# cgranerob/Land-Surface-Temperature-Super-Resolution-with-a-Scale-Invariance-Free-Neural-Approach

Measured on AMD Instinct MI355X. Metric: LST+NDVI 256x256 patches/sec (train fwd+bwd), whole job, higher is better.
Workload: dtype f32; 1 GPU; ModelB SIF-NN-SR2 (gradFTM loss) batch 64/GPU, synthetic 256x256, 1x MI355X, fwd+loss+bwd+Adam; batch_per_gpu=64, patch=256x256 (LST 64x64 + NDVI 256x256), parallelism=dp1, loss=sr2

## Files before the change

land-surface-temperature-super-resolution-with-a-scale-invariance-free-neural-approach_amd/csrc/resample.hip:

```cpp
#include "edge_conv.h"

namespace {

__device__ __forceinline__ float4 maybe_bnrelu(float4 v, const float* scale, const float* shift, int c) {
  return scale != nullptr ? bn_relu4(v, ld4(scale + c), ld4(shift + c)) : v;
}

template <bool HS>
__global__ void bnrelu_pool2_kernel(const float* __restrict__ y, const float* scale, const float* shift,
                                    float* __restrict__ out, int B, int H, int W, int C) {
  const unsigned Q = C / 4, Ho = H / 2, Wo = W / 2;
  const unsigned n = (unsigned)B * Ho * Wo * Q;
  for (unsigned e = blockIdx.x * blockDim.x + threadIdx.x; e < n; e += gridDim.x * blockDim.x) {
    const unsigned p = e / Q;
    const int c = (int)(e - p * Q) * 4;
    const unsigned rr = p / Wo, ox = p - rr * Wo, b = rr / Ho, oy = rr - b * Ho;
    const size_t s = (((size_t)b * H + 2 * oy) * W + 2 * ox) * C + c;
    const float4 v00 = maybe_bnrelu(ldA4<HS>(y, s), scale, shift, c), v01 = maybe_bnrelu(ldA4<HS>(y, s + C), scale, shift, c);
    const float4 v10 = maybe_bnrelu(ldA4<HS>(y, s + (size_t)W * C), scale, shift, c);
    const float4 v11 = maybe_bnrelu(ldA4<HS>(y, s + (size_t)W * C + C), scale, shift, c);
    float4 o;
    o.x = (v00.x + v01.x + v10.x + v11.x) * 0.25f;
    o.y = (v00.y + v01.y + v10.y + v11.y) * 0.25f;
    o.z = (v00.z + v01.z + v10.z + v11.z) * 0.25f;
    o.w = (v00.w + v01.w + v10.w + v11.w) * 0.25f;
    stA4<HS>(out, (size_t)p * C + c, o);
  }
}

template <bool HS>
__global__ void bnrelu_add_kernel(const float* __restrict__ p, const float* __restrict__ y, const float* scale,
                                  const float* shift, float* __restrict__ out, int C, size_t nquads) {
  const unsigned Q = C / 4;
  for (size_t e = (size_t)blockIdx.x * blockDim.x + threadIdx.x; e < nquads; e += (size_t)gridDim.x * blockDim.x) {
    const int c = (int)((unsigned)e % Q) * 4;
    const float4 a = ldA4<HS>(p, e * 4), v = maybe_bnrelu(ldA4<HS>(y, e * 4), scale, shift, c);
    stA4<HS>(out, e * 4, make_float4(a.x + v.x, a.y + v.y, a.z + v.z, a.w + v.w));
  }
}

__device__ __forceinline__ void up_coord(int o, int in, int out, int& i0, int& i1, float& l0, float& l1) {
#pragma clang fp contract(off)
  const float ratio = out > 1 ? (float)(in - 1) / (float)(out - 1) : 0.f;
  const float src = ratio * (float)o;
  i0 = (int)src;
  i1 = i0 + (i0 < in - 1 ? 1 : 0);
  l1 = src - (float)i0;
  l0 = 1.f - l1;
}

template <bool HS>
__global__ void bnrelu_up2x_kernel(const float* __restrict__ y, const float* scale, const float* shift,
                                   float* __restrict__ out, int B, int Hin, int Win, int C) {
  const int Q = C / 4, Ho = 2 * Hin, Wo = 2 * Win;
  const size_t n = (size_t)B * Ho * Wo * Q;
  for (size_t e = (size_t)blockIdx.x * blockDim.x + threadIdx.x; e < n; e += (size_t)gridDim.x * blockDim.x) {
    const int c = (int)(e % Q) * 4;
    const size_t p = e / Q;
    const int ox = p % Wo, oy = (p / Wo) % Ho, b = p / ((size_t)Wo * Ho);
    int y0, y1, x0, x1; float hy0, hy1, hx0, hx1;
    up_coord(oy, Hin, Ho, y0, y1, hy0, hy1);
    up_coord(ox, Win, Wo, x0, x1, hx0, hx1);
    const size_t base = (size_t)b * Hin * Win * C + c;
    const float4 v00 = maybe_bnrelu(ldA4<HS>(y, base + ((size_t)y0 * Win + x0) * C), scale, shift, c);
    const float4 v01 = maybe_bnrelu(ldA4<HS>(y, base + ((size_t)y0 * Win + x1) * C), scale, shift, c);
    const float4 v10 = maybe_bnrelu(ldA4<HS>(y, base + ((size_t)y1 * Win + x0) * C), scale, shift, c);
    const float4 v11 = maybe_bnrelu(ldA4<HS>(y, base + ((size_t)y1 * Win + x1) * C), scale, shift, c);
    float4 o;
    o.x = hy0 * (hx0 * v00.x + hx1 * v01.x) + hy1 * (hx0 * v10.x + hx1 * v11.x);
    o.y = hy0 * (hx0 * v00.y + hx1 * v01.y) + hy1 * (hx0 * v10.y + hx1 * v11.y);
    o.z = hy0 * (hx0 * v00.z + hx1 * v01.z) + hy1 * (hx0 * v10.z + hx1 * v11.z);
    o.w = hy0 * (hx0 * v00.w + hx1 * v01.w) + hy1 * (hx0 * v10.w + hx1 * v11.w);
    stA4<HS>(out, p * C + c, o);
  }
}

template <bool HS>
__global__ void pool2_bwd_kernel(const float* __restrict__ gp, float* __restrict__ g, int B, int H, int W, int C,
                                 int accumulate) {
  const int Q = C / 4, Ho = H / 2, Wo = W / 2;
  const size_t n = (size_t)B * H * W * Q;
  for (size_t e = (size_t)blockIdx.x * blockDim.x + threadIdx.x; e < n; e += (size_t)gridDim.x * blockDim.x) {
    const int c = (int)(e % Q) * 4;
    const size_t p = e / Q;
    const int x = p % W, yy = (p / W) % H, b = p / ((size_t)W * H);
    const float4 v = ldA4<HS>(gp, (((size_t)b * Ho + yy / 2) * Wo + x / 2) * C + c);
    float4 o = make_float4(0.25f * v.x, 0.25f * v.y, 0.25f * v.z, 0.25f * v.w);
    if (accumulate) {
      const float4 a = ldA4<HS>(g, p * C + c);
      o.x += a.x; o.y += a.y; o.z += a.z; o.w += a.w;
    }
    stA4<HS>(g, p * C + c, o);
  }
}

template <bool HS>
__global__ void up2x_bwd_kernel(const float* __restrict__ gu, float* __restrict__ g, int B, int Hin, int Win, int C) {
  SIFSR_CHAIN_PRIO();
  const int Q = C / 4, Ho = 2 * Hin, Wo = 2 * Win;
  const size_t n = (size_t)B * Hin * Win * Q;
  for (size_t e = (size_t)blockIdx.x * blockDim.x + threadIdx.x; e < n; e += (size_t)gridDim.x * blockDim.x) {
    const int c = (int)(e % Q) * 4;
    const size_t p = e / Q;
    const int ix = p % Win, iy = (p / Win) % Hin, b = p / ((size_t)Win * Hin);
    float wy[5], wx[5];
#pragma unroll
    for (int k = 0; k < 5; ++k) {
      const int oy = 2 * iy - 2 + k, ox = 2 * ix - 2 + k;
      wy[k] = 0.f; wx[k] = 0.f;
      if (oy >= 0 && oy < Ho) {
        int a0, a1; float l0, l1;
        up_coord(oy, Hin, Ho, a0, a1, l0, l1);
        wy[k] = (a0 == iy ? l0 : 0.f) + (a1 == iy ? l1 : 0.f);
      }
      if (ox >= 0 && ox < Wo) {
        int a0, a1; float l0, l1;
        up_coord(ox, Win, Wo, a0, a1, l0, l1);
        wx[k] = (a0 == ix ? l0 : 0.f) + (a1 == ix ? l1 : 0.f);
      }
    }
    float4 acc = make_float4(0.f, 0.f, 0.f, 0.f);
#pragma unroll
    for (int ky = 0; ky < 5; ++ky) {
      if (wy[ky] == 0.f) continue;
      const int oy = 2 * iy - 2 + ky;
#pragma unroll
      for (int kx = 0; kx < 5; ++kx) {
        if (wx[kx] == 0.f) continue;
        const int ox = 2 * ix - 2 + kx;
        const float w = wy[ky] * wx[kx];
        const float4 v = ldA4<HS>(gu, (((size_t)b * Ho + oy) * Wo + ox) * C + c);
        acc.x = fmaf(w, v.x, acc.x); acc.y = fmaf(w, v.y, acc.y); acc.z = fmaf(w, v.z, acc.z); acc.w = fmaf(w, v.w, acc.w);
      }
    }
    stA4<HS>(g, p * C + c, acc);
  }
}

template <int C, bool HS>
__global__ __launch_bounds__(256) void bnrelu_up2x_tile_kernel(const float* __restrict__ y, const float* scale,
                                                               const float* shift, float* __restrict__ out, int Hin,
                                                               int Win) {
  constexpr int Q = C / 4, SR = 10;
  __shared__ float4 src[SR * SR * Q];
  const int tid = threadIdx.x;
  const int Ho = 2 * Hin, Wo = 2 * Win;
  const int ox0 = blockIdx.x * 16, oy0 = blockIdx.y * 16, b = blockIdx.z;
  int sy0, sx0, t1; float f0, f1;
  up_coord(oy0, Hin, Ho, sy0, t1, f0, f1);
  up_coord(ox0, Win, Wo, sx0, t1, f0, f1);
  for (int e = tid; e < SR * SR * Q; e += 256) {
    const int c4 = e % Q, p = e / Q;
    const int py = p / SR, px = p - py * SR;
    const int gy = min(sy0 + py, Hin - 1), gx = min(sx0 + px, Win - 1);
    src[e] = maybe_bnrelu(ldA4<HS>(y, ((size_t)(b * Hin + gy) * Win + gx) * C + 4 * c4), scale, shift, 4 * c4);
  }
  __syncthreads();
  for (int e = tid; e < 256 * Q; e += 256) {
    const int c4 = e % Q, p = e / Q;
    const int oy = oy0 + (p >> 4), ox = ox0 + (p & 15);
    if (oy >= Ho || ox >= Wo) continue;
    int y0, y1, x0, x1; float hy0, hy1, hx0, hx1;
    up_coord(oy, Hin, Ho, y0, y1, hy0, hy1);
    up_coord(ox, Win, Wo, x0, x1, hx0, hx1);
    const float4 v00 = src[((y0 - sy0) * SR + (x0 - sx0)) * Q + c4], v01 = src[((y0 - sy0) * SR + (x1 - sx0)) * Q + c4];
    const float4 v10 = src[((y1 - sy0) * SR + (x0 - sx0)) * Q + c4], v11 = src[((y1 - sy0) * SR + (x1 - sx0)) * Q + c4];
    float4 o;
    o.x = hy0 * (hx0 * v00.x + hx1 * v01.x) + hy1 * (hx0 * v10.x + hx1 * v11.x);
    o.y = hy0 * (hx0 * v00.y + hx1 * v01.y) + hy1 * (hx0 * v10.y + hx1 * v11.y);
    o.z = hy0 * (hx0 * v00.z + hx1 * v01.z) + hy1 * (hx0 * v10.z + hx1 * v11.z);
    o.w = hy0 * (hx0 * v00.w + hx1 * v01.w) + hy1 * (hx0 * v10.w + hx1 * v11.w);
    stA4<HS>(out, ((size_t)(b * Ho + oy) * Wo + ox) * C + 4 * c4, o);
  }
}

template <int C, bool HS>
__global__ __launch_bounds__(256) void up2x_bwd_tile_kernel(const float* __restrict__ gu, float* __restrict__ g, int Hin,
                                                            int Win, const float* __restrict__ bn_y,
                                                            const float* __restrict__ bn_scale,
                                                            const float* __restrict__ bn_shift,
                                                            float* __restrict__ bn_partials) {
  SIFSR_CHAIN_PRIO();
  constexpr int TL = 8, HR = 2 * TL + 3, NCH = C / 16;
  __shared__ float4 hi[HR * HR * 4];
  __shared__ float4 tmp[HR * TL * 4];
  __shared__ float wxs[TL][5], wys[TL][5];
  const int tid = threadIdx.x;
  const int Ho = 2 * Hin, Wo = 2 * Win;
  const int ix0 = blockIdx.x * TL, iy0 = blockIdx.y * TL;
  const int b = blockIdx.z / NCH, ch0 = (blockIdx.z % NCH) * 16;
  if (tid < 2 * TL * 5) {
    const bool isy = tid >= TL * 5;
    const int t = isy ? tid - TL * 5 : tid;
    const int il = t / 5, k = t - il * 5;
    const int i = (isy ? iy0 : ix0) + il, in = isy ? Hin : Win, on = isy ? Ho : Wo;
    const int o = 2 * i - 2 + k;
    float w = 0.f;
    if (i < in && o >= 0 && o < on) {
      int a0, a1; float l0, l1;
      up_coord(o, in, on, a0, a1, l0, l1);
      w = (a0 == i ? l0 : 0.f) + (a1 == i ? l1 : 0.f);
    }
    if (isy) wys[il][k] = w; else wxs[il][k] = w;
  }
  for (int e = tid; e < HR * HR * 4; e += 256) {
    const int q = e & 3, p = e >> 2;
    const int py = p / HR, px = p - py * HR;
    const int oy = 2 * iy0 - 2 + py, ox = 2 * ix0 - 2 + px;
    float4 v = make_float4(0.f, 0.f, 0.f, 0.f);
    if (oy >= 0 && oy < Ho && ox >= 0 && ox < Wo) v = ldA4<HS>(gu, ((size_t)(b * Ho + oy) * Wo + ox) * C + ch0 + 4 * q);
    hi[e] = v;
  }
  __syncthreads();
  for (int e = tid; e < HR * TL * 4; e += 256) {
    const int q = e & 3, p = e >> 2;
    const int py = p / TL, il = p - py * TL;
    float4 acc = make_float4(0.f, 0.f, 0.f, 0.f);
#pragma unroll
    for (int k = 0; k < 5; ++k) {
      const float w = wxs[il][k];
      const float4 v = hi[(py * HR + 2 * il + k) * 4 + q];
      acc.x = fmaf(w, v.x, acc.x); acc.y = fmaf(w, v.y, acc.y); acc.z = fmaf(w, v.z, acc.z); acc.w = fmaf(w, v.w, acc.w);
    }
    tmp[e] = acc;
  }
  __syncthreads();
  {
    const int q = tid & 3, p = tid >> 2;
    const int il_y = p / TL, il_x = p - il_y * TL;
    const int iy = iy0 + il_y, ix = ix0 + il_x;
    float4 acc = make_float4(0.f, 0.f, 0.f, 0.f);
#pragma unroll
    for (int k = 0; k < 5; ++k) {
      const float w = wys[il_y][k];
      const float4 v = tmp[((2 * il_y + k) * TL + il_x) * 4 + q];
      acc.x = fmaf(w, v.x, acc.x); acc.y = fmaf(w, v.y, acc.y); acc.z = fmaf(w, v.z, acc.z); acc.w = fmaf(w, v.w, acc.w);
    }
    const bool in = iy < Hin && ix < Win;
    acc = as_stored4<HS>(acc);
    if (in) stA4<HS>(g, ((size_t)(b * Hin + iy) * Win + ix) * C + ch0 + 4 * q, acc);
    if (bn_partials != nullptr) {
      float4 d1 = make_float4(0.f, 0.f, 0.f, 0.f), d2 = d1;
      if (in) {
        const float4 yv = ldA4<HS>(bn_y, ((size_t)(b * Hin + iy) * Win + ix) * C + ch0 + 4 * q);
        const float4 sc = ld4(bn_scale + ch0 + 4 * q), sh = ld4(bn_shift + ch0 + 4 * q);
        d1.x = fmaf(yv.x, sc.x, sh.x) > 0.f ? acc.x : 0.f; d2.x = d1.x * yv.x;
        d1.y = fmaf(yv.y, sc.y, sh.y) > 0.f ? acc.y : 0.f; d2.y = d1.y * yv.y;
        d1.z = fmaf(yv.z, sc.z, sh.z) > 0.f ? acc.z : 0.f; d2.z = d1.z * yv.z;
        d1.w = fmaf(yv.w, sc.w, sh.w) > 0.f ? acc.w : 0.f; d2.w = d1.w * yv.w;
      }
      float v8[8] = {d1.x, d1.y, d1.z, d1.w, d2.x, d2.y, d2.z, d2.w};
#pragma unroll
      for (int m = 4; m < 64; m <<= 1)
#pragma unroll
        for (int j = 0; j < 8; ++j) v8[j] += __shfl_xor(v8[j], m);
      __syncthreads();
      float* const red = reinterpret_cast<float*>(hi);
      if ((tid & 63) < 4) {
#pragma unroll
        for (int j = 0; j < 8; ++j) red[((tid >> 6) * 4 + (tid & 3)) * 8 + j] = v8[j];
      }
      __syncthreads();
      if (tid < 32) {
        const int qq = tid & 3, r = (tid >> 2) & 3, which = tid >> 4;
        const float sum = (red[(0 * 4 + qq) * 8 + which * 4 + r] + red[(1 * 4 + qq) * 8 + which * 4 + r]) +
                          (red[(2 * 4 + qq) * 8 + which * 4 + r] + red[(3 * 4 + qq) * 8 + which * 4 + r]);
        const size_t row = ((size_t)b * gridDim.y + blockIdx.y) * gridDim.x + blockIdx.x;
        bn_partials[(row * C + ch0 + 4 * qq + r) * 2 + which] = sum;
      }
    }
  }
}

inline int grid_for(size_t n) {
  size_t b = (n + 255) / 256;
  return (int)(b > 16384 ? 16384 : (b < 1 ? 1 : b));
}

}

int launch_bnrelu_pool2(const float* y, const float* scale, const float* shift, float* out, int B, int H, int W, int C, hipStream_t s) {
  if (H % 2 || W % 2 || C % 4 || (size_t)B * H * W * C >= ((size_t)1 << 32)) return SIFSR_ERR_SHAPE;
  if (sifsr_half_storage()) hipLaunchKernelGGL(bnrelu_pool2_kernel<true>, dim3(grid_for((size_t)B * H / 2 * W / 2 * C / 4)), dim3(256), 0, s, y, scale, shift, out, B, H, W, C);
  else hipLaunchKernelGGL(bnrelu_pool2_kernel<false>, dim3(grid_for((size_t)B * H / 2 * W / 2 * C / 4)), dim3(256), 0, s, y, scale, shift, out, B, H, W, C);
  SIFSR_LAUNCH_CHECK();
  return SIFSR_OK;
}
int launch_bnrelu_add(const float* p, const float* y, const float* scale, const float* shift, float* out, int C, size_t npix, hipStream_t s) {
  if (C % 4) return SIFSR_ERR_SHAPE;
  const size_t nq = npix * C / 4;
  if (sifsr_half_storage()) hipLaunchKernelGGL(bnrelu_add_kernel<true>, dim3(grid_for(nq)), dim3(256), 0, s, p, y, scale, shift, out, C, nq);
  else hipLaunchKernelGGL(bnrelu_add_kernel<false>, dim3(grid_for(nq)), dim3(256), 0, s, p, y, scale, shift, out, C, nq);
  SIFSR_LAUNCH_CHECK();
  return SIFSR_OK;
}
int launch_bnrelu_up2x(const float* y, const float* scale, const float* shift, float* out, int B, int Hin, int Win, int C, hipStream_t s) {
  if (C % 4) return SIFSR_ERR_SHAPE;
  if ((C == 16 || C == 32 || C == 64) && B <= 65535 && Hin >= 2 && Win >= 2) {
    const dim3 grid((2 * Win + 15) / 16, (2 * Hin + 15) / 16, B);
#define SIFSR_UP(CV, HV) hipLaunchKernelGGL((bnrelu_up2x_tile_kernel<CV, HV>), grid, dim3(256), 0, s, y, scale, shift, out, Hin, Win)
    const bool hs = sifsr_half_storage();
    if (C == 16) { if (hs) SIFSR_UP(16, true); else SIFSR_UP(16, false); }
    else if (C == 32) { if (hs) SIFSR_UP(32, true); else SIFSR_UP(32, false); }
    else { if (hs) SIFSR_UP(64, true); else SIFSR_UP(64, false); }
#undef SIFSR_UP
    SIFSR_LAUNCH_CHECK();
    return SIFSR_OK;
  }
  if (sifsr_half_storage()) hipLaunchKernelGGL(bnrelu_up2x_kernel<true>, dim3(grid_for((size_t)B * Hin * Win * C)), dim3(256), 0, s, y, scale, shift, out, B, Hin, Win, C);
  else hipLaunchKernelGGL(bnrelu_up2x_kernel<false>, dim3(grid_for((size_t)B * Hin * Win * C)), dim3(256), 0, s, y, scale, shift, out, B, Hin, Win, C);
  SIFSR_LAUNCH_CHECK();
  return SIFSR_OK;
}
int launch_pool2_bwd(const float* gp, float* g, int B, int H, int W, int C, int accumulate, hipStream_t s) {
  if (H % 2 || W % 2 || C % 4) return SIFSR_ERR_SHAPE;
  if (sifsr_half_storage()) hipLaunchKernelGGL(pool2_bwd_kernel<true>, dim3(grid_for((size_t)B * H * W * C / 4)), dim3(256), 0, s, gp, g, B, H, W, C, accumulate);
  else hipLaunchKernelGGL(pool2_bwd_kernel<false>, dim3(grid_for((size_t)B * H * W * C / 4)), dim3(256), 0, s, gp, g, B, H, W, C, accumulate);
  SIFSR_LAUNCH_CHECK();
  return SIFSR_OK;
}
int up2x_bwd_stat_rows(int B, int Hin, int Win, int C) {
  if (!((C == 16 || C == 32 || C == 64) && (size_t)B * (C / 16) <= 65535)) return 0;
  return B * ((Hin + 7) / 8) * ((Win + 7) / 8);
}

int launch_up2x_bwd(const float* gu, float* g, int B, int Hin, int Win, int C, hipStream_t s, const float* bn_y,
                    const float* bn_scale, const float* bn_shift, float* bn_partials) {
  if (C % 4) return SIFSR_ERR_SHAPE;
  if (bn_partials != nullptr && (!bn_y || !bn_scale || !bn_shift || up2x_bwd_stat_rows(B, Hin, Win, C) == 0)) return SIFSR_ERR_ARG;
  if ((C == 16 || C == 32 || C == 64) && (size_t)B * (C / 16) <= 65535) {
    const dim3 grid((Win + 7) / 8, (Hin + 7) / 8, B * (C / 16));
#define SIFSR_UPB(CV, HV) hipLaunchKernelGGL((up2x_bwd_tile_kernel<CV, HV>), grid, dim3(256), 0, s, gu, g, Hin, Win, bn_y, bn_scale, bn_shift, bn_partials)
    const bool hs = sifsr_half_storage();
    if (C == 16) { if (hs) SIFSR_UPB(16, true); else SIFSR_UPB(16, false); }
    else if (C == 32) { if (hs) SIFSR_UPB(32, true); else SIFSR_UPB(32, false); }
    else { if (hs) SIFSR_UPB(64, true); else SIFSR_UPB(64, false); }
#undef SIFSR_UPB
    SIFSR_LAUNCH_CHECK();
    return SIFSR_OK;
  }
  if (sifsr_half_storage()) hipLaunchKernelGGL(up2x_bwd_kernel<true>, dim3(grid_for((size_t)B * Hin * Win * C / 4)), dim3(256), 0, s, gu, g, B, Hin, Win, C);
  else hipLaunchKernelGGL(up2x_bwd_kernel<false>, dim3(grid_for((size_t)B * Hin * Win * C / 4)), dim3(256), 0, s, gu, g, B, Hin, Win, C);
  SIFSR_LAUNCH_CHECK();
  return SIFSR_OK;
}
```

Baseline: 10750 patches/s.

## Make up2x backward tile kernel persistent with software-pipelined tile prefetch

```diff
diff --git a/land-surface-temperature-super-resolution-with-a-scale-invariance-free-neural-approach_amd/csrc/resample.hip b/land-surface-temperature-super-resolution-with-a-scale-invariance-free-neural-approach_amd/csrc/resample.hip
--- a/land-surface-temperature-super-resolution-with-a-scale-invariance-free-neural-approach_amd/csrc/resample.hip
+++ b/land-surface-temperature-super-resolution-with-a-scale-invariance-free-neural-approach_amd/csrc/resample.hip
@@ -1,4 +1,6 @@
 #include "edge_conv.h"
+#include <algorithm>
+#include <type_traits>
 
 namespace {
 
@@ -174,102 +176,223 @@
   }
 }
 
-template <int C, bool HS>
-__global__ __launch_bounds__(256) void up2x_bwd_tile_kernel(const float* __restrict__ gu, float* __restrict__ g, int Hin,
-                                                            int Win, const float* __restrict__ bn_y,
-                                                            const float* __restrict__ bn_scale,
-                                                            const float* __restrict__ bn_shift,
-                                                            float* __restrict__ bn_partials) {
-  SIFSR_CHAIN_PRIO();
-  constexpr int TL = 8, HR = 2 * TL + 3, NCH = C / 16;
-  __shared__ float4 hi[HR * HR * 4];
-  __shared__ float4 tmp[HR * TL * 4];
-  __shared__ float wxs[TL][5], wys[TL][5];
+#ifndef SIFSR_UP2X_WGS
+#define SIFSR_UP2X_WGS 1024
+#endif
+#ifndef SIFSR_UP2X_WALK_MIN
+#define SIFSR_UP2X_WALK_MIN 4
+#endif
+#ifndef SIFSR_UP2X_WALK_MAX
+#define SIFSR_UP2X_WALK_MAX 16
+#endif
+#ifndef SIFSR_UP2X_LDS_PAD
+#define SIFSR_UP2X_LDS_PAD 0
+#endif
+
+template <bool HS> struct RawQuad { using type = float4; };
+template <> struct RawQuad<true> { using type = uint2; };
+template <bool HS> static __device__ __forceinline__ typename RawQuad<HS>::type ld_raw4(const float* base, size_t e) {
+  if constexpr (HS) return *reinterpret_cast<const uint2*>(reinterpret_cast<const unsigned short*>(base) + e);
+  else return *reinterpret_cast<const float4*>(base + e);
+}
+template <bool HS> static __device__ __forceinline__ float4 widen4(typename RawQuad<HS>::type r) {
+  if constexpr (HS) return unpack_bf16x4(r); else return r;
+}
+
+static __device__ __forceinline__ int fresh(int v) { asm volatile("" : "+v"(v)); return v; }
+
+template <int C> struct Up2xBwdLds {
+  static constexpr int HI = 6 * 256, TMP = 19 * 8 * 4, YB = 256, BNC = 2 * (C / 4);
+  static constexpr size_t BYTES = (size_t)(HI + TMP + YB + BNC) * sizeof(float4) + (4 * 8 * 5 + 4 * 4 * 8) * sizeof(float);
+};
+
+template <int C, bool HS, bool STATS>
+__device__ __forceinline__ void up2x_bwd_walk(const float* __restrict__ gu, float* __restrict__ g, int Hin, int Win,
+                                              const float* __restrict__ bn_y, const float* __restrict__ bn_scale,
+                                              const float* __restrict__ bn_shift, float* __restrict__ bn_partials,
+                                              int n_items, int walk) {
+  constexpr int TL = 8, HR = 2 * TL + 3, NCH = C / 16, NW = HR * HR * 4, NLD = (NW + 255) / 256;
+  using Raw = typename RawQuad<HS>::type;
+  extern __shared__ float4 up2x_bwd_lds[];
+  using Lds = Up2xBwdLds<C>;
+  float4* const hi = up2x_bwd_lds;
+  float4* const tmp = hi + Lds::HI;
+  float4* const yb = tmp + Lds::TMP;
+  float4 (*const bnc)[C / 4] = reinterpret_cast<float4 (*)[C / 4]>(yb + Lds::YB);
+  float* const fl = reinterpret_cast<float*>(yb + Lds::YB + Lds::BNC);
+  float (*const wxs)[TL][5] = reinterpret_cast<float (*)[TL][5]>(fl);
+  float (*const wys)[TL][5] = wxs + 2;
+  float* const red = fl + 4 * TL * 5;
   const int tid = threadIdx.x;
   const int Ho = 2 * Hin, Wo = 2 * Win;
-  const int ix0 = blockIdx.x * TL, iy0 = blockIdx.y * TL;
-  const int b = blockIdx.z / NCH, ch0 = (blockIdx.z % NCH) * 16;
-  if (tid < 2 * TL * 5) {
-    const bool isy = tid >= TL * 5;
-    const int t = isy ? tid - TL * 5 : tid;
-    const int il = t / 5, k = t - il * 5;
-    const int i = (isy ? iy0 : ix0) + il, in = isy ? Hin : Win, on = isy ? Ho : Wo;
-    const int o = 2 * i - 2 + k;
-    float w = 0.f;
-    if (i < in && o >= 0 && o < on) {
-      int a0, a1; float l0, l1;
-      up_coord(o, in, on, a0, a1, l0, l1);
-      w = (a0 == i ? l0 : 0.f) + (a1 == i ? l1 : 0.f);
-    }
-    if (isy) wys[il][k] = w; else wxs[il][k] = w;
-  }
-  for (int e = tid; e < HR * HR * 4; e += 256) {
-    const int q = e & 3, p = e >> 2;
-    const int py = p / HR, px = p - py * HR;
-    const int oy = 2 * iy0 - 2 + py, ox = 2 * ix0 - 2 + px;
-    float4 v = make_float4(0.f, 0.f, 0.f, 0.f);
-    if (oy >= 0 && oy < Ho && ox >= 0 && ox < Wo) v = ldA4<HS>(gu, ((size_t)(b * Ho + oy) * Wo + ox) * C + ch0 + 4 * q);
-    hi[e] = v;
-  }
+  const int tiles_x = (Win + TL - 1) / TL, tiles_y = (Hin + TL - 1) / TL;
+  const int n0 = blockIdx.x * walk, n1 = min(n0 + walk, n_items);
+  constexpr bool stats = STATS;
+  if (stats && tid < C / 4) { bnc[0][tid] = ld4(bn_scale + 4 * tid); bnc[1][tid] = ld4(bn_shift + 4 * tid); }
+
+  struct Item { int b, iy0, ix0, ch0, row; };
+  auto item_of = [&](int n) {
+    Item it;
+    it.row = n / NCH; it.ch0 = (n - it.row * NCH) * 16;
+    const int r = it.row / tiles_x;
+    it.ix0 = (it.row - r * tiles_x) * TL;
+    it.b = r / tiles_y;
+    it.iy0 = (r - it.b * tiles_y) * TL;
+    return it;
+  };
+  auto issue = [&](const Item& it, Raw (&r)[NLD], unsigned& ok) {
+    ok = 0;
+    const int tv = fresh(tid);
+#pragma unroll
+    for (int k = 0; k < NLD; ++k) {
+      const int e = tv + 256 * k, ec = min(e, NW - 1);
+      const int q = ec & 3, p = ec >> 2;
+      const int py = p / HR, px = p - py * HR;
+      const int oy = 2 * it.iy0 - 2 + py, ox = 2 * it.ix0 - 2 + px;
+      ok |= (unsigned)((e < NW) & (oy >= 0) & (oy < Ho) & (ox >= 0) & (ox < Wo)) << k;
+      r[k] = ld_raw4<HS>(gu, ((size_t)(it.b * Ho + clampi(oy, 0, Ho - 1)) * Wo + clampi(ox, 0, Wo - 1)) * C + it.ch0 + 4 * q);
+      __builtin_amdgcn_sched_barrier(0);
+    }
+    ok = (unsigned)fresh((int)ok);
+  };
+  auto land = [&](const Raw (&r)[NLD], unsigned ok) {
+    const int tv = fresh(tid);
+#pragma unroll
+    for (int k = 0; k < NLD; ++k) {
+      hi[tv + 256 * k] = (ok >> k) & 1u ? widen4<HS>(r[k]) : make_float4(0.f, 0.f, 0.f, 0.f);
+    }
+  };
+  auto issue_y = [&](const Item& it) {
+    const int tv = fresh(tid);
+    const int q = tv & 3, p = tv >> 2;
+    const int iy = min(it.iy0 + p / TL, Hin - 1), ix = min(it.ix0 + (p & (TL - 1)), Win - 1);
+    return ld_raw4<HS>(bn_y, ((size_t)(it.b * Hin + iy) * Win + ix) * C + it.ch0 + 4 * q);
+  };
+  auto weights = [&](const Item& it, int slot) {
+    const int tv = fresh(tid);
+    if (tv < 2 * TL * 5) {
+      const bool isy = tv >= TL * 5;
+      const int t = isy ? tv - TL * 5 : tv;
+      const int il = t / 5, k = t - il * 5;
+      const int i = (isy ? it.iy0 : it.ix0) + il, in = isy ? Hin : Win, on = isy ? Ho : Wo;
+      const int o = 2 * i - 2 + k;
+      float w = 0.f;
+      if (i < in && o >= 0 && o < on) {
+        int a0, a1; float l0, l1;
+        up_coord(o, in, on, a0, a1, l0, l1);
+        w = (a0 == i ? l0 : 0.f) + (a1 == i ? l1 : 0.f);
+      }
+      if (isy) wys[slot][il][k] = w; else wxs[slot][il][k] = w;
+    }
+  };
+
+  Raw win[NLD], y_next = Raw();
+  unsigned ok;
+  Item cur = item_of(n0);
+  weights(cur, 0);
+  issue(cur, win, ok);
+  if constexpr (stats) y_next = issue_y(cur);
+  land(win, ok);
+  if constexpr (stats) yb[tid] = widen4<HS>(y_next);
   __syncthreads();
-  for (int e = tid; e < HR * TL * 4; e += 256) {
-    const int q = e & 3, p = e >> 2;
-    const int py = p / TL, il = p - py * TL;
+  auto step = [&](auto more_c, int n) {
+    constexpr bool more = decltype(more_c)::value;
+    const int slot = (n - n0) & 1;
+    Item nxt = cur;
+    if constexpr (more) {
+      nxt = item_of(n + 1);
+      weights(nxt, slot ^ 1);
+      issue(nxt, win, ok);
+      if constexpr (stats) y_next = issue_y(nxt);
+      __builtin_amdgcn_sched_barrier(0);
+    }
+#pragma unroll 1
+    for (int e = fresh(tid); e < HR * TL * 4; e += 256) {
+      const int q = e & 3, p = e >> 2;
+      const int py = p / TL, il = p - py * TL;
+      float4 acc = make_float4(0.f, 0.f, 0.f, 0.f);
+#pragma unroll
+      for (int k = 0; k < 5; ++k) {
+        const float w = wxs[slot][il][k];
+        const float4 v = hi[(py * HR + 2 * il + k) * 4 + q];
+        acc.x = fmaf(w, v.x, acc.x); acc.y = fmaf(w, v.y, acc.y); acc.z = fmaf(w, v.z, acc.z); acc.w = fmaf(w, v.w, acc.w);
+        if (k == 2) __builtin_amdgcn_sched_barrier(0);
+      }
+      tmp[e] = acc;
+    }
+    __syncthreads();
     float4 acc = make_float4(0.f, 0.f, 0.f, 0.f);
-#pragma unroll
-    for (int k = 0; k < 5; ++k) {
-      const float w = wxs[il][k];
-      const float4 v = hi[(py * HR + 2 * il + k) * 4 + q];
-      acc.x = fmaf(w, v.x, acc.x); acc.y = fmaf(w, v.y, acc.y); acc.z = fmaf(w, v.z, acc.z); acc.w = fmaf(w, v.w, acc.w);
-    }
-    tmp[e] = acc;
-  }
-  __syncthreads();
-  {
-    const int q = tid & 3, p = tid >> 2;
-    const int il_y = p / TL, il_x = p - il_y * TL;
-    const int iy = iy0 + il_y, ix = ix0 + il_x;
-    float4 acc = make_float4(0.f, 0.f, 0.f, 0.f);
-#pragma unroll
-    for (int k = 0; k < 5; ++k) {
-      const float w = wys[il_y][k];
-      const float4 v = tmp[((2 * il_y + k) * TL + il_x) * 4 + q];
-      acc.x = fmaf(w, v.x, acc.x); acc.y = fmaf(w, v.y, acc.y); acc.z = fmaf(w, v.z, acc.z); acc.w = fmaf(w, v.w, acc.w);
-    }
-    const bool in = iy < Hin && ix < Win;
-    acc = as_stored4<HS>(acc);
-    if (in) stA4<HS>(g, ((size_t)(b * Hin + iy) * Win + ix) * C + ch0 + 4 * q, acc);
-    if (bn_partials != nullptr) {
-      float4 d1 = make_float4(0.f, 0.f, 0.f, 0.f), d2 = d1;
-      if (in) {
-        const float4 yv = ldA4<HS>(bn_y, ((size_t)(b * Hin + iy) * Win + ix) * C + ch0 + 4 * q);
-        const float4 sc = ld4(bn_scale + ch0 + 4 * q), sh = ld4(bn_shift + ch0 + 4 * q);
-        d1.x = fmaf(yv.x, sc.x, sh.x) > 0.f ? acc.x : 0.f; d2.x = d1.x * yv.x;
-        d1.y = fmaf(yv.y, sc.y, sh.y) > 0.f ? acc.y : 0.f; d2.y = d1.y * yv.y;
-        d1.z = fmaf(yv.z, sc.z, sh.z) > 0.f ? acc.z : 0.f; d2.z = d1.z * yv.z;
-        d1.w = fmaf(yv.w, sc.w, sh.w) > 0.f ? acc.w : 0.f; d2.w = d1.w * yv.w;
-      }
-      float v8[8] = {d1.x, d1.y, d1.z, d1.w, d2.x, d2.y, d2.z, d2.w};
+    float v8[8] = {0.f, 0.f, 0.f, 0.f, 0.f, 0.f, 0.f, 0.f};
+    {
+      const int tv = fresh(tid);
+      const int q = tv & 3, p = tv >> 2;
+      const int il_y = p / TL, il_x = p - il_y * TL;
+#pragma unroll
+      for (int k = 0; k < 5; ++k) {
+        const float w = wys[slot][il_y][k];
+        const float4 v = tmp[((2 * il_y + k) * TL + il_x) * 4 + q];
+        acc.x = fmaf(w, v.x, acc.x); acc.y = fmaf(w, v.y, acc.y); acc.z = fmaf(w, v.z, acc.z); acc.w = fmaf(w, v.w, acc.w);
+        if (k == 2) __builtin_amdgcn_sched_barrier(0);
+      }
+      acc = as_stored4<HS>(acc);
+      __builtin_amdgcn_sched_barrier(0);
+      if constexpr (stats) {
+        if (cur.iy0 + il_y < Hin && cur.ix0 + il_x < Win) {
+          const float4 yv = yb[tv];
+          const float4 sc = bnc[0][cur.ch0 / 4 + q], sh = bnc[1][cur.ch0 / 4 + q];
+          v8[0] = fmaf(yv.x, sc.x, sh.x) > 0.f ? acc.x : 0.f; v8[4] = v8[0] * yv.x;
+          v8[1] = fmaf(yv.y, sc.y, sh.y) > 0.f ? acc.y : 0.f; v8[5] = v8[1] * yv.y;
+          v8[2] = fmaf(yv.z, sc.z, sh.z) > 0.f ? acc.z : 0.f; v8[6] = v8[2] * yv.z;
+          v8[3] = fmaf(yv.w, sc.w, sh.w) > 0.f ? acc.w : 0.f; v8[7] = v8[3] * yv.w;
+        }
+      }
+    }
+    __builtin_amdgcn_sched_barrier(0);
+    if constexpr (more) {
+      land(win, ok);
+      if constexpr (stats) yb[tid] = widen4<HS>(y_next);
+    }
+    {
+      const int tv = fresh(tid);
+      const int q = tv & 3, p = tv >> 2;
+      const int iy = cur.iy0 + p / TL, ix = cur.ix0 + (p & (TL - 1));
+      if (iy < Hin && ix < Win) stA4<HS>(g, ((size_t)(cur.b * Hin + iy) * Win + ix) * C + cur.ch0 + 4 * q, acc);
+    }
+    __builtin_amdgcn_sched_barrier(0);
+    if constexpr (stats) {
 #pragma unroll
       for (int m = 4; m < 64; m <<= 1)
 #pragma unroll
         for (int j = 0; j < 8; ++j) v8[j] += __shfl_xor(v8[j], m);
-      __syncthreads();
-      float* const red = reinterpret_cast<float*>(hi);
-      if ((tid & 63) < 4) {
-#pragma unroll
-        for (int j = 0; j < 8; ++j) red[((tid >> 6) * 4 + (tid & 3)) * 8 + j] = v8[j];
-      }
-      __syncthreads();
-      if (tid < 32) {
-        const int qq = tid & 3, r = (tid >> 2) & 3, which = tid >> 4;
-        const float sum = (red[(0 * 4 + qq) * 8 + which * 4 + r] + red[(1 * 4 + qq) * 8 + which * 4 + r]) +
-                          (red[(2 * 4 + qq) * 8 + which * 4 + r] + red[(3 * 4 + qq) * 8 + which * 4 + r]);
-        const size_t row = ((size_t)b * gridDim.y + blockIdx.y) * gridDim.x + blockIdx.x;
-        bn_partials[(row * C + ch0 + 4 * qq + r) * 2 + which] = sum;
-      }
-    }
-  }
+      const int tv = fresh(tid);
+      if ((tv & 63) < 4) {
+#pragma unroll
+        for (int j = 0; j < 8; ++j) red[((tv >> 6) * 4 + (tv & 3)) * 8 + j] = v8[j];
+      }
+    }
+    __syncthreads();
+    if (stats && tid < 32) {
+      const int tv = fresh(tid);
+      const int qq = tv & 3, r = (tv >> 2) & 3, which = tv >> 4;
+      const float sum = (red[(0 * 4 + qq) * 8 + which * 4 + r] + red[(1 * 4 + qq) * 8 + which * 4 + r]) +
+                        (red[(2 * 4 + qq) * 8 + which * 4 + r] + red[(3 * 4 + qq) * 8 + which * 4 + r]);
+      bn_partials[((size_t)cur.row * C + cur.ch0 + 4 * qq + r) * 2 + which] = sum;
+    }
+    cur = nxt;
+  };
+  for (int n = n0; n + 1 < n1; ++n) step(std::true_type(), n);
+  step(std::false_type(), n1 - 1);
+}
+
+template <int C, bool HS>
+__global__ __launch_bounds__(256, 8) void up2x_bwd_tile_kernel(const float* __restrict__ gu, float* __restrict__ g, int Hin,
+                                                               int Win, const float* __restrict__ bn_y,
+                                                               const float* __restrict__ bn_scale,
+                                                               const float* __restrict__ bn_shift,
+                                                               float* __restrict__ bn_partials, int n_items, int walk) {
+  SIFSR_CHAIN_PRIO();
+  if (bn_partials != nullptr) up2x_bwd_walk<C, HS, true>(gu, g, Hin, Win, bn_y, bn_scale, bn_shift, bn_partials, n_items, walk);
+  else up2x_bwd_walk<C, HS, false>(gu, g, Hin, Win, bn_y, bn_scale, bn_shift, bn_partials, n_items, walk);
 }
 
 inline int grid_for(size_t n) {
@@ -329,8 +452,22 @@
   if (C % 4) return SIFSR_ERR_SHAPE;
   if (bn_partials != nullptr && (!bn_y || !bn_scale || !bn_shift || up2x_bwd_stat_rows(B, Hin, Win, C) == 0)) return SIFSR_ERR_ARG;
   if ((C == 16 || C == 32 || C == 64) && (size_t)B * (C / 16) <= 65535) {
-    const dim3 grid((Win + 7) / 8, (Hin + 7) / 8, B * (C / 16));
-#define SIFSR_UPB(CV, HV) hipLaunchKernelGGL((up2x_bwd_tile_kernel<CV, HV>), grid, dim3(256), 0, s, gu, g, Hin, Win, bn_y, bn_scale, bn_shift, bn_partials)
+    const size_t items = (size_t)B * ((Hin + 7) / 8) * ((Win + 7) / 8) * (C / 16);
+    if (items == 0 || items > (size_t)INT32_MAX - SIFSR_UP2X_WALK_MAX) return SIFSR_ERR_SHAPE;
+    const int n_items = (int)items;
+    const int walk = std::min(std::max(n_items / SIFSR_UP2X_WGS, SIFSR_UP2X_WALK_MIN), SIFSR_UP2X_WALK_MAX);
+    const dim3 grid((n_items + walk - 1) / walk);
+#if SIFSR_UP2X_LDS_PAD > 0
+#define SIFSR_UPB(CV, HV)                                                                                                         \
+  do {                                                                                                                            \
+    (void)hipFuncSetAttribute(reinterpret_cast<const void*>(&up2x_bwd_tile_kernel<CV, HV>), hipFuncAttributeMaxDynamicSharedMemorySize, \
+                              (int)(Up2xBwdLds<CV>::BYTES + SIFSR_UP2X_LDS_PAD));                                               \
+    hipLaunchKernelGGL((up2x_bwd_tile_kernel<CV, HV>), grid, dim3(256), Up2xBwdLds<CV>::BYTES + SIFSR_UP2X_LDS_PAD, s, gu, g, Hin, \
+                       Win, bn_y, bn_scale, bn_shift, bn_partials, n_items, walk);                                                \
+  } while (0)
+#else
+#define SIFSR_UPB(CV, HV) hipLaunchKernelGGL((up2x_bwd_tile_kernel<CV, HV>), grid, dim3(256), Up2xBwdLds<CV>::BYTES, s, gu, g, Hin, Win, bn_y, bn_scale, bn_shift, bn_partials, n_items, walk)
+#endif
     const bool hs = sifsr_half_storage();
     if (C == 16) { if (hs) SIFSR_UPB(16, true); else SIFSR_UPB(16, false); }
     else if (C == 32) { if (hs) SIFSR_UPB(32, true); else SIFSR_UPB(32, false); }
```

After: 10800 patches/s, median of 6. About the same (+0.5%).
